# mahak/khipu

Measured on AMD Instinct MI355X. Metric: node-hashes/sec (full state root, 100M-account trie), higher is better.
Workload: dtype u64

## Files before the change

### __graft_entry__.py

```python
import os
import subprocess
import sys

ROOT = os.path.dirname(os.path.abspath(__file__))
CSRC = os.path.join(ROOT, "khipu_amd", "csrc")
LIB = os.path.join(ROOT, "khipu_amd", "libkhst.so")
HIPCC = os.environ.get("HIPCC", "/opt/rocm/bin/hipcc")
HIP_FLAGS = ["--offload-arch=gfx950", "-O3", "-std=c++17", "-fPIC", "-Wall", "-Wno-unused-function",
             "-Wno-unknown-pragmas"]
UNITS = [("khst.hip", ["-falign-loops=64"]), ("leaf_kernel.hip", []), ("export_kernels.hip", []),
         ("prove_kernels.hip", []), ("load_kernels.hip", []), ("range_kernels.hip", []),
         ("rangeverify_kernels.hip", [])]
OBJ_DIR = os.path.join(ROOT, "build")

GENESIS_ROOT = "d7f8974fb5ac78d9ac099b9ad5018bedc2ce0a72dad1827a1709da30580f0544"


def _sources():
    return [os.path.join(CSRC, f) for f in sorted(os.listdir(CSRC)) if f.endswith((".hip", ".h"))] + [
        os.path.join(ROOT, "include", "khst.h")]


def build_lib(force=False, out=None, csrc=None, defines=()):
    out = out or LIB
    csrc = csrc or CSRC
    srcs = _sources()
    if out == LIB and not force and os.path.exists(LIB) and all(os.path.getmtime(LIB) >= os.path.getmtime(s) for s in srcs):
        return LIB
    os.makedirs(OBJ_DIR, exist_ok=True)
    tag = os.path.basename(out).replace(".so", "")
    procs, objs = [], []
    for src, extra in UNITS:
        obj = os.path.join(OBJ_DIR, f"{tag}_{src.replace('.hip', '.o')}")
        objs.append(obj)
        procs.append(subprocess.Popen([HIPCC] + HIP_FLAGS + extra + list(defines) + ["-c", "-o", obj,
                                                                                   os.path.join(csrc, src)], cwd=ROOT))
    if any(p.wait() for p in procs):
        raise subprocess.CalledProcessError(1, "hipcc (libkhst units)")
    subprocess.check_call([HIPCC, "--offload-arch=gfx950", "-shared", "-fPIC", "-o", out] + objs, cwd=ROOT)
    return out


CHECK_PROGRAMS = [
    ("xlane_check", "tests/test_gpu_parity.py::test_lane_spread_keccak_on_device"),
    ("prims_check", "tests/test_gpu_prims.py and tests/test_prims_plan.py"),
]


def build_check(name):
    src = os.path.join(ROOT, "scripts", name + ".hip")
    exe = os.path.join(ROOT, "scripts", name)
    deps = [src] + [os.path.join(CSRC, f) for f in os.listdir(CSRC) if f.endswith(".h")]
    if os.path.exists(exe) and all(os.path.getmtime(exe) >= os.path.getmtime(d) for d in deps):
        return
    subprocess.check_call([HIPCC, "--offload-arch=gfx950", "-O3", "-std=c++17", "-o", exe, src], cwd=ROOT)


def build() -> None:
    build_lib()
    for name, needed_by in CHECK_PROGRAMS:
        try:
            build_check(name)
        except (subprocess.CalledProcessError, OSError) as e:
            print(f"build: scripts/{name} not built ({e}); {needed_by} will fail", file=sys.stderr)
    subprocess.check_call(["make", "-s", "-C", os.path.join(ROOT, "oracle")])
    subprocess.check_call(["make", "-s", "-C", os.path.join(ROOT, "tests", "emu")])
    subprocess.check_call(["make", "-s", "-C", os.path.join(ROOT, "tests", "loopback")])
    sys.path.insert(0, ROOT)
    import khipu_amd
    khipu_amd.lib()
    subprocess.check_call(["make", "-s", "-C", os.path.join(ROOT, "tests", "jni_stub")])


def _genesis_inputs():
    sys.path.insert(0, ROOT)
    from khipu_amd import codec
    addrs, vals = [], []
    with open(os.path.join(ROOT, "tests", "golden", "genesis_alloc.txt")) as f:
        for line in f:
            a, b = line.split()
            addrs.append(bytes.fromhex(a))
            vals.append(codec.account_rlp(0, int(b)))
    return addrs, vals


def smoke() -> None:
    sys.path.insert(0, ROOT)
    import torch
    assert torch.cuda.is_available(), "smoke() needs a GPU"
    torch.cuda.set_device(0)
    import khipu_amd
    from oracle import oracle
    assert khipu_amd.lib().kh_device_count() >= 1
    addrs, vals = _genesis_inputs()
    st = khipu_amd.KhStats()
    root = khipu_amd.trie_root(addrs, vals, hash_keys=True, stats=st)
    assert root.hex() == GENESIS_ROOT, root.hex()
    import random
    rnd = random.Random(7)
    keys = [bytes(rnd.getrandbits(8) for _ in range(32)) for _ in range(300)]
    svals = [bytes([rnd.randrange(1, 0x80)]) for _ in keys]
    assert khipu_amd.trie_root(keys, svals) == oracle.seq_root(keys, svals)
    print(f"smoke ok: genesis root {root.hex()} ({st.n_node_hashes} node hashes, {st.t_total_ms:.3f} ms device)")


if __name__ == "__main__":
    {"build": build, "smoke": smoke}[sys.argv[1] if len(sys.argv) > 1 else "build"]()
```

### khipu_amd/csrc/prims.h

```cpp
#pragma once
#include <hip/hip_runtime.h>
#include <stdint.h>

#include "wave.h"

namespace khst {

constexpr int SCAN_THREADS = 256;
constexpr int SCAN_ITEMS = 8;
constexpr int SCAN_TILE = SCAN_THREADS * SCAN_ITEMS;

template <typename T>
__device__ __forceinline__ T block_exclusive_scan(T v, T* lds_waves, T* total) {
  const int lane = threadIdx.x & 63, w = threadIdx.x >> 6;
  T x = v;
#pragma unroll
  for (int o = 1; o < 64; o <<= 1) {
    T y = __shfl_up(x, o);
    if (lane >= o) x += y;
  }
  if (lane == 63) lds_waves[w] = x;
  __syncthreads();
  T wbase = 0, tot = 0;
#pragma unroll
  for (int i = 0; i < SCAN_THREADS / 64; ++i) {
    T s = lds_waves[i];
    if (i < w) wbase += s;
    tot += s;
  }
  __syncthreads();
  *total = tot;
  return wbase + x - v;
}

__device__ __forceinline__ uint64_t scan_n(uint64_t n, const uint32_t* n_dev) {
  return n_dev && (uint64_t)*n_dev < n ? (uint64_t)*n_dev : n;
}

template <typename T>
__global__ void __launch_bounds__(SCAN_THREADS) k_scan_tiles(const T* in, T* out, uint64_t n, T* tile_sums,
                                                             T* last_in, const uint32_t* n_dev) {
  topo_prio();
  n = scan_n(n, n_dev);
  __shared__ T lw[SCAN_THREADS / 64];
  uint64_t base = (uint64_t)blockIdx.x * SCAN_TILE + (uint64_t)threadIdx.x * SCAN_ITEMS;
  T v[SCAN_ITEMS];
  T s = 0;
#pragma unroll
  for (int i = 0; i < SCAN_ITEMS; ++i) {
    v[i] = (base + i < n) ? in[base + i] : (T)0;
    if (last_in && base + i == n - 1) *last_in = v[i];
    s += v[i];
  }
  T tot;
  T ex = block_exclusive_scan<T>(s, lw, &tot);
#pragma unroll
  for (int i = 0; i < SCAN_ITEMS; ++i) {
    if (base + i < n) out[base + i] = ex;
    ex += v[i];
  }
  if (threadIdx.x == 0) tile_sums[blockIdx.x] = tot;
}

template <typename T>
__global__ void __launch_bounds__(SCAN_THREADS) k_scan_add(T* out, uint64_t n, const T* tile_off,
                                                           const uint32_t* n_dev) {
  topo_prio();
  n = scan_n(n, n_dev);
  uint64_t base = (uint64_t)blockIdx.x * SCAN_TILE;
  if (base >= n) return;
  T add = tile_off[blockIdx.x];
  for (int i = threadIdx.x; i < SCAN_TILE; i += SCAN_THREADS)
    if (base + i < n) out[base + i] += add;
}

template <typename T>
__global__ void k_scan_total(const T* in_last, const T* out, uint64_t n, T* total, const uint32_t* n_dev) {
  topo_prio();
  n = scan_n(n, n_dev);
  *total = n ? *in_last + out[n - 1] : (T)0;
}

constexpr int SCAN_SMALL_THREADS = 1024;
constexpr uint64_t SCAN_SMALL_MAX = 32768;
template <typename T>
__device__ __forceinline__ void scan_small_block(const T* in, T* out, uint64_t n, T* total) {
  constexpr int IT = sizeof(T) == 8 ? 4 : 8;
  constexpr uint32_t TILE = SCAN_SMALL_THREADS * IT;
  __shared__ T buf[TILE + TILE / 32];
  __shared__ T lw[SCAN_SMALL_THREADS / 64];
  const uint32_t tid = threadIdx.x;
  const int lane = tid & 63, w = tid >> 6;
  T carry = 0;
  T v[IT];
  auto load = [&](uint64_t t0) {
#pragma unroll
    for (int i = 0; i < IT; ++i) {
      const uint64_t idx = t0 + (uint64_t)i * SCAN_SMALL_THREADS + tid;
      v[i] = idx < n ? in[idx] : (T)0;
    }
  };
  auto at = [](uint32_t p) { return p + (p >> 5); };
  load(0);
  for (uint64_t t0 = 0; t0 < n; t0 += TILE) {
#pragma unroll
    for (int i = 0; i < IT; ++i) buf[at(i * SCAN_SMALL_THREADS + tid)] = v[i];
    __syncthreads();
    if (t0 + TILE < n) load(t0 + TILE);
    T cur[IT];
    T s = 0;
#pragma unroll
    for (int j = 0; j < IT; ++j) {
      cur[j] = buf[at(tid * IT + j)];
      s += cur[j];
    }
    T x = s;
#pragma unroll
    for (int o = 1; o < 64; o <<= 1) {
      T y = __shfl_up(x, o);
      if (lane >= o) x += y;
    }
    if (lane == 63) lw[w] = x;
    __syncthreads();
    T wbase = 0, tot = 0;
#pragma unroll
    for (int i = 0; i < SCAN_SMALL_THREADS / 64; ++i) {
      const T q = lw[i];
      if (i < w) wbase += q;
      tot += q;
    }
    T ex = carry + wbase + x - s;
#pragma unroll
    for (int j = 0; j < IT; ++j) {
      buf[at(tid * IT + j)] = ex;
      ex += cur[j];
    }
    __syncthreads();
#pragma unroll
    for (int i = 0; i < IT; ++i) {
      const uint32_t p = i * SCAN_SMALL_THREADS + tid;
      if (t0 + p < n) out[t0 + p] = buf[at(p)];
    }
    carry += tot;
    __syncthreads();
  }
  if (total && tid == 0) *total = carry;
}
template <typename T>
__global__ void __launch_bounds__(SCAN_SMALL_THREADS) k_scan_small(const T* in, T* out, uint64_t n, T* total) {
  topo_prio();
  scan_small_block<T>(in, out, n, total);
}
struct ScanJob {
  const void* in;
  void* out;
  void* total;
  bool wide;
};
__global__ void __launch_bounds__(SCAN_SMALL_THREADS) k_scan_small3(ScanJob a, ScanJob b, ScanJob c, uint64_t n) {
  topo_prio();
  const ScanJob& j = blockIdx.x == 0 ? a : blockIdx.x == 1 ? b : c;
  if (!j.in) return;
  if (j.wide)
    scan_small_block<uint64_t>((const uint64_t*)j.in, (uint64_t*)j.out, n, (uint64_t*)j.total);
  else
    scan_small_block<uint32_t>((const uint32_t*)j.in, (uint32_t*)j.out, n, (uint32_t*)j.total);
}

constexpr uint64_t SCAN_TWO_MAX_TILES = 2048;
template <typename T>
__global__ void __launch_bounds__(SCAN_THREADS) k_scan_add_sums(T* out, uint64_t n, const T* sums, uint32_t tiles,
                                                                T* total, const uint32_t* n_dev) {
  topo_prio();
  n = scan_n(n, n_dev);
  __shared__ T lw[SCAN_THREADS / 64];
  const uint32_t b = blockIdx.x;
  T s = 0;
  for (uint32_t t = threadIdx.x; t < b; t += SCAN_THREADS) s += sums[t];
  s = wave_sum(s);
  if ((threadIdx.x & 63) == 0) lw[threadIdx.x >> 6] = s;
  __syncthreads();
  T add = 0;
#pragma unroll
  for (int i = 0; i < SCAN_THREADS / 64; ++i) add += lw[i];
  const uint64_t base = (uint64_t)b * SCAN_TILE;
  if (add)
    for (int i = threadIdx.x; i < SCAN_TILE; i += SCAN_THREADS)
      if (base + i < n) out[base + i] += add;
  if (total && b == tiles - 1 && threadIdx.x == 0) *total = add + sums[b];
}

inline size_t scan_scratch_bytes(uint64_t n, size_t elem) {
  size_t b = 0;
  while (n > 1) {
    n = (n + SCAN_TILE - 1) / SCAN_TILE;
    b += ((n + 1) * elem + 63) / 64 * 64 + 64;
  }
  return b + 128;
}

template <typename T>
void scan_exclusive(const T* in, T* out, uint64_t n, T* total, void* scratch, hipStream_t st, bool small_ok = true,
                    const uint32_t* n_dev = nullptr) {
  if (n == 0) {
    if (total) (void)hipMemsetAsync(total, 0, sizeof(T), st);
    return;
  }
  if (small_ok && !n_dev && n <= SCAN_SMALL_MAX) {
    hipLaunchKernelGGL(k_scan_small<T>, dim3(1), dim3(SCAN_SMALL_THREADS), 0, st, in, out, n, total);
    return;
  }
  uint64_t tiles = (n + SCAN_TILE - 1) / SCAN_TILE;
  T* sums = (T*)scratch;
  T* last_in = sums + tiles;
  if (tiles <= SCAN_TWO_MAX_TILES) {
    hipLaunchKernelGGL(k_scan_tiles<T>, dim3((unsigned)tiles), dim3(SCAN_THREADS), 0, st, in, out, n, sums,
                       (T*)nullptr, n_dev);
    hipLaunchKernelGGL(k_scan_add_sums<T>, dim3((unsigned)tiles), dim3(SCAN_THREADS), 0, st, out, n, (const T*)sums,
                       (uint32_t)tiles, total, n_dev);
    return;
  }
  hipLaunchKernelGGL(k_scan_tiles<T>, dim3((unsigned)tiles), dim3(SCAN_THREADS), 0, st, in, out, n, sums,
                     total ? last_in : (T*)nullptr, n_dev);
  if (tiles > 1) {
    char* next = (char*)scratch + (((tiles + 1) * sizeof(T) + 63) / 64) * 64 + 64;
    scan_exclusive<T>(sums, sums, tiles, (T*)nullptr, next, st, false);
    hipLaunchKernelGGL(k_scan_add<T>, dim3((unsigned)tiles), dim3(SCAN_THREADS), 0, st, out, n, (const T*)sums,
                       n_dev);
  }
  if (total)
    hipLaunchKernelGGL(k_scan_total<T>, dim3(1), dim3(1), 0, st, (const T*)last_in, (const T*)out, n, total, n_dev);
}

constexpr int RS_THREADS = 256;
#ifndef KHST_RS_ITEMS
#define KHST_RS_ITEMS 16
#endif
constexpr int RS_ITEMS = KHST_RS_ITEMS;
constexpr int RS_TILE = RS_THREADS * RS_ITEMS;
constexpr int RS_WAVES = RS_THREADS / 64;
constexpr int RS_MAX_PASSES = 8;
constexpr unsigned long long RS_ST_AGG = 1ull << 62, RS_ST_INC = 2ull << 62, RS_ST_CNT = RS_ST_AGG - 1;
constexpr size_t RS_HDR_BYTES = (RS_MAX_PASSES * 256 + RS_MAX_PASSES) * sizeof(uint32_t);
constexpr size_t RS_HDR_PAD = (RS_HDR_BYTES + 255) / 256 * 256;

template <typename K, int IT>
__global__ void __launch_bounds__(RS_THREADS) k_rs_hist_all(const K* keys, uint64_t n, int lo_bit, int npass,
                                                            uint32_t* ghist, unsigned long long* st0, uint64_t nst) {
  constexpr int TILE = RS_THREADS * IT;
  __shared__ uint32_t h[RS_MAX_PASSES][256];
  for (int i = threadIdx.x; i < RS_MAX_PASSES * 256; i += RS_THREADS) (&h[0][0])[i] = 0;
  for (uint64_t i = (uint64_t)blockIdx.x * RS_THREADS + threadIdx.x; i < nst; i += (uint64_t)gridDim.x * RS_THREADS)
    st0[i] = 0;
  __syncthreads();
  for (uint64_t t0 = (uint64_t)blockIdx.x * TILE; t0 < n; t0 += (uint64_t)gridDim.x * TILE) {
    K kk[IT];
#pragma unroll
    for (int it = 0; it < IT; ++it) {
      const uint64_t i = t0 + (uint64_t)it * RS_THREADS + threadIdx.x;
      kk[it] = keys[i < n ? i : n - 1];
    }
#pragma unroll
    for (int it = 0; it < IT; ++it) {
      if (t0 + (uint64_t)it * RS_THREADS + threadIdx.x < n)
        for (int p = 0; p < npass; ++p) atomicAdd(&h[p][(uint32_t)(kk[it] >> (lo_bit + 8 * p)) & 0xFF], 1u);
    }
  }
  __syncthreads();
  for (int i = threadIdx.x; i < npass * 256; i += RS_THREADS) {
    const uint32_t v = (&h[0][0])[i];
    if (v) atomicAdd(&ghist[i], v);
  }
}

template <typename K, int IT = RS_ITEMS>
__global__ void __launch_bounds__(RS_THREADS) k_rs_pass(const K* keys, const uint32_t* vals, K* okeys,
                                                        uint32_t* ovals, uint64_t n, int shift, const uint32_t* ghist,
                                                        unsigned long long* status, unsigned long long* status_next,
                                                        uint32_t* ticket) {
  constexpr int TILE = RS_THREADS * IT, WSLICE = TILE / RS_WAVES;
  __shared__ uint32_t wc[RS_WAVES][256];
  __shared__ uint32_t tstart[256], gbase[256];
  __shared__ uint32_t lw[RS_THREADS / 64];
  __shared__ uint32_t s_tile;
  __shared__ K sk[TILE];
  __shared__ uint32_t sv[TILE];
  const int w = threadIdx.x >> 6, lane = threadIdx.x & 63;
  if (threadIdx.x == 0) s_tile = atomicAdd(ticket, 1u);
  const uint32_t gtot = ghist[threadIdx.x];
  if (status_next) status_next[(uint64_t)blockIdx.x * 256 + threadIdx.x] = 0;
  for (int i = threadIdx.x; i < RS_WAVES * 256; i += RS_THREADS) (&wc[0][0])[i] = 0;
  __syncthreads();
  const uint32_t tile = s_tile;
  const uint64_t tbase = (uint64_t)tile * TILE;
  const uint64_t base = tbase + (uint64_t)w * WSLICE;
  K k[IT];
  uint32_t v[IT];
  uint32_t r[IT];
  const uint64_t lt = lanemask_lt();
#pragma unroll
  for (int it = 0; it < IT; ++it) {
    uint64_t i = base + (uint64_t)it * 64 + lane;
    bool valid = i < n;
    k[it] = valid ? keys[i] : 0;
    v[it] = valid ? vals[i] : 0;
  }
#pragma unroll
  for (int it = 0; it < IT; ++it) {
    uint64_t i = base + (uint64_t)it * 64 + lane;
    bool valid = i < n;
    uint32_t d = (uint32_t)(k[it] >> shift) & 0xFF;
    uint64_t peers = __ballot(valid);
#pragma unroll
    for (int b = 0; b < 8; ++b) {
      bool bit = (d >> b) & 1;
      uint64_t bb = __ballot(bit);
      peers &= bit ? bb : ~bb;
    }
    uint32_t cnt = valid ? wc[w][d] : 0;
    uint32_t below = (uint32_t)__popcll(peers & lt);
    r[it] = cnt + below;
    if (valid && below == 0) wc[w][d] = cnt + (uint32_t)__popcll(peers);
    __builtin_amdgcn_wave_barrier();
  }
  __syncthreads();
  {
    const int d = threadIdx.x;
    uint32_t run = 0;
#pragma unroll
    for (int q = 0; q < RS_WAVES; ++q) {
      uint32_t t = wc[q][d];
      wc[q][d] = run;
      run += t;
    }
    unsigned long long* my = status + (uint64_t)tile * 256 + d;
    __hip_atomic_store(my, (tile == 0 ? RS_ST_INC : RS_ST_AGG) | run, __ATOMIC_RELAXED, __HIP_MEMORY_SCOPE_AGENT);
    uint32_t tot;
    tstart[d] = block_exclusive_scan<uint32_t>(run, lw, &tot);
    const uint32_t dbase = block_exclusive_scan<uint32_t>(gtot, lw, &tot);
    uint64_t excl = 0;
    if (tile > 0) {
      for (uint64_t t = tile - 1;;) {
        const unsigned long long s =
            __hip_atomic_load(status + t * 256 + d, __ATOMIC_RELAXED, __HIP_MEMORY_SCOPE_AGENT);
        if ((s >> 62) == 0) {
          __builtin_amdgcn_s_sleep(1);
          continue;
        }
        excl += s & RS_ST_CNT;
        if ((s >> 62) == 2) break;
        --t;
      }
      __hip_atomic_store(my, RS_ST_INC | (excl + run), __ATOMIC_RELAXED, __HIP_MEMORY_SCOPE_AGENT);
    }
    gbase[d] = dbase + (uint32_t)excl;
  }
  __syncthreads();
#pragma unroll
  for (int it = 0; it < IT; ++it) {
    uint64_t i = base + (uint64_t)it * 64 + lane;
    if (i < n) {
      uint32_t d = (uint32_t)(k[it] >> shift) & 0xFF;
      uint32_t li = tstart[d] + wc[w][d] + r[it];
      sk[li] = k[it];
      sv[li] = v[it];
    }
  }
  __syncthreads();
  const uint32_t tn = (uint32_t)((n - tbase) < (uint64_t)TILE ? (n - tbase) : (uint64_t)TILE);
  for (uint32_t li = threadIdx.x; li < tn; li += RS_THREADS) {
    K key = sk[li];
    uint32_t d = (uint32_t)(key >> shift) & 0xFF;
    uint32_t pos = gbase[d] + (li - tstart[d]);
    okeys[pos] = key;
    ovals[pos] = sv[li];
  }
}

constexpr int RS_SMALL_ITEMS = 4;
constexpr uint64_t RS_SMALL_N = 65536;
#ifndef KHST_RS_BIG_ITEMS
#define KHST_RS_BIG_ITEMS 32
#endif
constexpr int RS_BIG_ITEMS = KHST_RS_BIG_ITEMS;
constexpr uint64_t RS_BIG_N = 1ull << 22;
inline int radix_items(uint64_t n, size_t key_bytes) {
  return n <= RS_SMALL_N ? RS_SMALL_ITEMS : (n >= RS_BIG_N && key_bytes == 4) ? RS_BIG_ITEMS : RS_ITEMS;
}
inline uint64_t radix_tiles(uint64_t n, size_t key_bytes) {
  const uint64_t tile = (uint64_t)RS_THREADS * (uint64_t)radix_items(n, key_bytes);
  return (n + tile - 1) / tile;
}
inline size_t radix_scratch_bytes(uint64_t n) {
  return RS_HDR_PAD + 2 * radix_tiles(n, 8) * 256 * sizeof(unsigned long long) + 256;
}

template <typename K>
inline bool radix_sort_pairs(K* k0, uint32_t* v0, K* k1, uint32_t* v1, uint64_t n, int lo_bit, int hi_bit,
                             void* scratch, hipStream_t st, bool hdr_zeroed = false) {
  if (n <= 1 || hi_bit <= lo_bit) return false;
  const int items = radix_items(n, sizeof(K));
  const uint64_t tiles = radix_tiles(n, sizeof(K));
  const int npass = (hi_bit - lo_bit + 7) / 8;
  uint32_t* ghist = (uint32_t*)scratch;
  uint32_t* ticket = ghist + RS_MAX_PASSES * 256;
  unsigned long long* stat[2] = {(unsigned long long*)((char*)scratch + RS_HDR_PAD), nullptr};
  stat[1] = stat[0] + tiles * 256;
  if (!hdr_zeroed) (void)hipMemsetAsync(ghist, 0, RS_HDR_BYTES, st);
  const unsigned hgrid = (unsigned)(tiles < 1024 ? tiles : 1024);
  if (items == RS_SMALL_ITEMS)
    hipLaunchKernelGGL((k_rs_hist_all<K, RS_SMALL_ITEMS>), dim3(hgrid), dim3(RS_THREADS), 0, st, (const K*)k0, n,
                       lo_bit, npass, ghist, stat[0], tiles * 256);
  else
    hipLaunchKernelGGL((k_rs_hist_all<K, RS_ITEMS>), dim3(hgrid), dim3(RS_THREADS), 0, st, (const K*)k0, n, lo_bit,
                       npass, ghist, stat[0], tiles * 256);
  bool flip = false;
  for (int p = 0; p < npass; ++p) {
    K* ik = flip ? k1 : k0;
    uint32_t* iv = flip ? v1 : v0;
    K* ok = flip ? k0 : k1;
    uint32_t* ov = flip ? v0 : v1;
    unsigned long long* nxt = p + 1 < npass ? stat[(p + 1) & 1] : nullptr;
    if (items == RS_SMALL_ITEMS)
      hipLaunchKernelGGL((k_rs_pass<K, RS_SMALL_ITEMS>), dim3((unsigned)tiles), dim3(RS_THREADS), 0, st, (const K*)ik,
                         (const uint32_t*)iv, ok, ov, n, lo_bit + 8 * p, (const uint32_t*)(ghist + 256 * p), stat[p & 1],
                         nxt, ticket + p);
    else if (sizeof(K) == 4 && items == RS_BIG_ITEMS)
      hipLaunchKernelGGL((k_rs_pass<K, sizeof(K) == 4 ? RS_BIG_ITEMS : RS_ITEMS>), dim3((unsigned)tiles), dim3(RS_THREADS), 0, st, (const K*)ik,
                         (const uint32_t*)iv, ok, ov, n, lo_bit + 8 * p, (const uint32_t*)(ghist + 256 * p), stat[p & 1],
                         nxt, ticket + p);
    else
      hipLaunchKernelGGL((k_rs_pass<K>), dim3((unsigned)tiles), dim3(RS_THREADS), 0, st, (const K*)ik,
                         (const uint32_t*)iv, ok, ov, n, lo_bit + 8 * p, (const uint32_t*)(ghist + 256 * p), stat[p & 1],
                         nxt, ticket + p);
    flip = !flip;
  }
  return flip;
}

}
```

Before: 3.634 billion.

## Restructure radix scatter pass to share key/value LDS and defer value loads

Rewrites the onesided radix sort pass: keys and values now share one LDS buffer, with keys scattered first and values reloaded and scattered in a second phase. Value loads are deferred until after the look-back. Per-item ranks pack the digit so tstart can be dropped, and full slices use unpredicated loads. The kernel gets a waves_per_eu hint and scalarised wave/tile indices. The aim is to cut LDS footprint for higher occupancy and to overlap the global loads with the decoupled look-back, at the cost of an extra barrier phase and re-reading digits. It also adds optional look-back statistics and a new check program.

```diff
diff --git a/__graft_entry__.py b/__graft_entry__.py
--- a/__graft_entry__.py
+++ b/__graft_entry__.py
@@ -44,6 +44,7 @@
 CHECK_PROGRAMS = [
     ("xlane_check", "tests/test_gpu_parity.py::test_lane_spread_keccak_on_device"),
     ("prims_check", "tests/test_gpu_prims.py and tests/test_prims_plan.py"),
+    ("radix_pass_check", "tests/test_gpu_radix_pass.py"),
 ]
 
 
diff --git a/khipu_amd/csrc/prims.h b/khipu_amd/csrc/prims.h
--- a/khipu_amd/csrc/prims.h
+++ b/khipu_amd/csrc/prims.h
@@ -273,42 +273,53 @@
   }
 }
 
+template <typename T, int IT>
+__device__ __forceinline__ void rs_load_slice(T (&dst)[IT], const T* src, uint64_t base, uint64_t lbase,
+                                              uint32_t llast, bool full, int lane) {
+  if (full) {
+    const T* p = src + base + lane;
+#pragma unroll
+    for (int it = 0; it < IT; ++it) dst[it] = p[it * 64];
+  } else {
+#pragma unroll
+    for (int it = 0; it < IT; ++it) {
+      const uint32_t o = (uint32_t)it * 64 + lane;
+      dst[it] = src[lbase + (o < llast ? o : llast)];
+    }
+  }
+}
+
 template <typename K, int IT = RS_ITEMS>
-__global__ void __launch_bounds__(RS_THREADS) k_rs_pass(const K* keys, const uint32_t* vals, K* okeys,
-                                                        uint32_t* ovals, uint64_t n, int shift, const uint32_t* ghist,
-                                                        unsigned long long* status, unsigned long long* status_next,
-                                                        uint32_t* ticket) {
+__global__ void __launch_bounds__(RS_THREADS) __attribute__((amdgpu_waves_per_eu(4)))
+k_rs_pass(const K* keys, const uint32_t* vals, K* okeys, uint32_t* ovals, uint64_t n, int shift, const uint32_t* ghist,
+          unsigned long long* status, unsigned long long* status_next, uint32_t* ticket) {
   constexpr int TILE = RS_THREADS * IT, WSLICE = TILE / RS_WAVES;
   __shared__ uint32_t wc[RS_WAVES][256];
-  __shared__ uint32_t tstart[256], gbase[256];
+  __shared__ uint32_t gbase[256];
   __shared__ uint32_t lw[RS_THREADS / 64];
   __shared__ uint32_t s_tile;
   __shared__ K sk[TILE];
-  __shared__ uint32_t sv[TILE];
-  const int w = threadIdx.x >> 6, lane = threadIdx.x & 63;
+  uint32_t* const sv = (uint32_t*)sk;
+  const int w = __builtin_amdgcn_readfirstlane(threadIdx.x >> 6), lane = threadIdx.x & 63;
   if (threadIdx.x == 0) s_tile = atomicAdd(ticket, 1u);
   const uint32_t gtot = ghist[threadIdx.x];
   if (status_next) status_next[(uint64_t)blockIdx.x * 256 + threadIdx.x] = 0;
   for (int i = threadIdx.x; i < RS_WAVES * 256; i += RS_THREADS) (&wc[0][0])[i] = 0;
   __syncthreads();
-  const uint32_t tile = s_tile;
+  const uint32_t tile = __builtin_amdgcn_readfirstlane(s_tile);
   const uint64_t tbase = (uint64_t)tile * TILE;
   const uint64_t base = tbase + (uint64_t)w * WSLICE;
   K k[IT];
   uint32_t v[IT];
   uint32_t r[IT];
   const uint64_t lt = lanemask_lt();
+  const uint32_t wn = base < n ? (uint32_t)((n - base) < (uint64_t)WSLICE ? (n - base) : (uint64_t)WSLICE) : 0u;
+  const uint64_t lbase = wn ? base : tbase;
+  const uint32_t llast = wn ? wn - 1 : 0u;
+  rs_load_slice<K, IT>(k, keys, base, lbase, llast, wn == (uint32_t)WSLICE, lane);
 #pragma unroll
   for (int it = 0; it < IT; ++it) {
-    uint64_t i = base + (uint64_t)it * 64 + lane;
-    bool valid = i < n;
-    k[it] = valid ? keys[i] : 0;
-    v[it] = valid ? vals[i] : 0;
-  }
-#pragma unroll
-  for (int it = 0; it < IT; ++it) {
-    uint64_t i = base + (uint64_t)it * 64 + lane;
-    bool valid = i < n;
+    bool valid = lane < (int)wn - it * 64;
     uint32_t d = (uint32_t)(k[it] >> shift) & 0xFF;
     uint64_t peers = __ballot(valid);
 #pragma unroll
@@ -319,61 +330,107 @@
     }
     uint32_t cnt = valid ? wc[w][d] : 0;
     uint32_t below = (uint32_t)__popcll(peers & lt);
-    r[it] = cnt + below;
+    r[it] = (cnt + below) + (d << 16);
+    asm volatile("" : "+v"(r[it]));
     if (valid && below == 0) wc[w][d] = cnt + (uint32_t)__popcll(peers);
     __builtin_amdgcn_wave_barrier();
   }
   __syncthreads();
+  const int dt = threadIdx.x;
+  uint32_t run = 0, ts, dbase;
+  unsigned long long* const my = status + (uint64_t)tile * 256 + dt;
   {
-    const int d = threadIdx.x;
-    uint32_t run = 0;
+    const int d = dt;
+    uint32_t wcnt[RS_WAVES];
 #pragma unroll
     for (int q = 0; q < RS_WAVES; ++q) {
-      uint32_t t = wc[q][d];
-      wc[q][d] = run;
-      run += t;
-    }
-    unsigned long long* my = status + (uint64_t)tile * 256 + d;
+      wcnt[q] = wc[q][d];
+      run += wcnt[q];
+    }
     __hip_atomic_store(my, (tile == 0 ? RS_ST_INC : RS_ST_AGG) | run, __ATOMIC_RELAXED, __HIP_MEMORY_SCOPE_AGENT);
     uint32_t tot;
-    tstart[d] = block_exclusive_scan<uint32_t>(run, lw, &tot);
-    const uint32_t dbase = block_exclusive_scan<uint32_t>(gtot, lw, &tot);
+    ts = block_exclusive_scan<uint32_t>(run, lw, &tot);
+    dbase = block_exclusive_scan<uint32_t>(gtot, lw, &tot);
+    uint32_t ws = ts;
+#pragma unroll
+    for (int q = 0; q < RS_WAVES; ++q) {
+      wc[q][d] = ws;
+      ws += wcnt[q];
+    }
+  }
+  __syncthreads();
+#pragma unroll
+  for (int it = 0; it < IT; ++it) {
+    if (lane < (int)wn - it * 64) {
+      r[it] = (r[it] & 0xFFFF) + wc[w][r[it] >> 16];
+      sk[r[it]] = k[it];
+    }
+  }
+  {
+    const int d = dt;
     uint64_t excl = 0;
     if (tile > 0) {
+#ifdef KHST_RS_LOOKBACK_STATS
+      unsigned long long st_words = 0, st_rounds = 0;
+#endif
       for (uint64_t t = tile - 1;;) {
         const unsigned long long s =
             __hip_atomic_load(status + t * 256 + d, __ATOMIC_RELAXED, __HIP_MEMORY_SCOPE_AGENT);
+#ifdef KHST_RS_LOOKBACK_STATS
+        ++st_rounds;
+#endif
         if ((s >> 62) == 0) {
           __builtin_amdgcn_s_sleep(1);
           continue;
         }
+#ifdef KHST_RS_LOOKBACK_STATS
+        ++st_words;
+#endif
         excl += s & RS_ST_CNT;
         if ((s >> 62) == 2) break;
         --t;
       }
       __hip_atomic_store(my, RS_ST_INC | (excl + run), __ATOMIC_RELAXED, __HIP_MEMORY_SCOPE_AGENT);
-    }
-    gbase[d] = dbase + (uint32_t)excl;
-  }
-  __syncthreads();
-#pragma unroll
-  for (int it = 0; it < IT; ++it) {
-    uint64_t i = base + (uint64_t)it * 64 + lane;
-    if (i < n) {
-      uint32_t d = (uint32_t)(k[it] >> shift) & 0xFF;
-      uint32_t li = tstart[d] + wc[w][d] + r[it];
-      sk[li] = k[it];
-      sv[li] = v[it];
-    }
-  }
+#ifdef KHST_RS_LOOKBACK_STATS
+      {
+        const long p = (RS_MAX_PASSES * 256 - (long)(ticket - ghist)) / 255;
+        unsigned long long* sw = (unsigned long long*)((char*)(ghist - 256 * p) + RS_HDR_BYTES) + 3 * p;
+        atomicAdd(sw, st_words);
+        atomicAdd(sw + 1, st_rounds);
+        atomicMax(sw + 2, st_words);
+      }
+#endif
+    }
+    gbase[d] = dbase + (uint32_t)excl - ts;
+  }
+  rs_load_slice<uint32_t, IT>(v, vals, base, lbase, llast, wn == (uint32_t)WSLICE, lane);
   __syncthreads();
   const uint32_t tn = (uint32_t)((n - tbase) < (uint64_t)TILE ? (n - tbase) : (uint64_t)TILE);
-  for (uint32_t li = threadIdx.x; li < tn; li += RS_THREADS) {
-    K key = sk[li];
-    uint32_t d = (uint32_t)(key >> shift) & 0xFF;
-    uint32_t pos = gbase[d] + (li - tstart[d]);
-    okeys[pos] = key;
-    ovals[pos] = sv[li];
+  uint32_t dg[(IT + 3) / 4];
+#pragma unroll
+  for (int j = 0; j < (IT + 3) / 4; ++j) dg[j] = 0;
+#pragma unroll
+  for (int j = 0; j < IT; ++j) {
+    const uint32_t li = threadIdx.x + (uint32_t)j * RS_THREADS;
+    if (li < tn) {
+      K key = sk[li];
+      uint32_t d = (uint32_t)(key >> shift) & 0xFF;
+      dg[j / 4] |= d << (8 * (j % 4));
+      okeys[gbase[d] + li] = key;
+    }
+  }
+  __syncthreads();
+#pragma unroll
+  for (int it = 0; it < IT; ++it)
+    if (lane < (int)wn - it * 64) sv[r[it]] = v[it];
+  __syncthreads();
+#pragma unroll
+  for (int j = 0; j < IT; ++j) {
+    const uint32_t li = threadIdx.x + (uint32_t)j * RS_THREADS;
+    if (li < tn) {
+      uint32_t d = (dg[j / 4] >> (8 * (j % 4))) & 0xFF;
+      ovals[gbase[d] + li] = sv[li];
+    }
   }
 }
 
@@ -407,6 +464,10 @@
   unsigned long long* stat[2] = {(unsigned long long*)((char*)scratch + RS_HDR_PAD), nullptr};
   stat[1] = stat[0] + tiles * 256;
   if (!hdr_zeroed) (void)hipMemsetAsync(ghist, 0, RS_HDR_BYTES, st);
+#ifdef KHST_RS_LOOKBACK_STATS
+  static_assert(RS_HDR_BYTES % 8 == 0 && RS_HDR_BYTES + RS_MAX_PASSES * 24 <= RS_HDR_PAD, "look-back statistics");
+  (void)hipMemsetAsync((char*)scratch + RS_HDR_BYTES, 0, RS_MAX_PASSES * 24, st);
+#endif
   const unsigned hgrid = (unsigned)(tiles < 1024 ? tiles : 1024);
   if (items == RS_SMALL_ITEMS)
     hipLaunchKernelGGL((k_rs_hist_all<K, RS_SMALL_ITEMS>), dim3(hgrid), dim3(RS_THREADS), 0, st, (const K*)k0, n,
```

Result: no change. 3.646 billion (median of 2 runs) (+0.3%).
